# kianoosh-j/CL_MultiView_Stereo

Hardware: AMD Instinct MI355X
Metric: Mpix/s depth (1080p, 128 depth hyp, 5 views) + depth L1 vs ref (higher is better)
Workload: dtype i8 (NCC: 8-bit intensities as int8 v_dot4 operands, i32 window sums, f32 costs; SLIC / superpixel SAD / refinement in f32 with the reference's f64 promotions)

## Files before the change

cl_multiview_stereo_amd/csrc/launch_plan.cpp:

```cpp
#include "launch_plan.h"

#include <algorithm>
#include <climits>
#include <cmath>
#include <cstdlib>
#include <cstring>

extern char** environ;

namespace mvs {
namespace plan {

Tuning plan_tuning() {
  Tuning t;
  bool any = false;
  for (char** e = environ; e && *e && !any; e++) {
    const char* s = *e;
    any = s[0] == 'M' && s[1] == 'V' && s[2] == 'S' && s[3] == '_' && (s[4] == 'S' || s[4] == 'F');
  }
  if (!any) return t;
  const auto num = [](const char* name, int dflt) {
    const char* e = getenv(name);
    return e ? atoi(e) : dflt;
  };
  const auto is = [](const char* name, const char* value) {
    const char* e = getenv(name);
    return e && !strcmp(e, value);
  };
  const int wps = num("MVS_SWEEP_WPS", 0);
  t.sweep_wps = (wps == 1 || wps == 2 || wps == 4) ? wps : 0;
  t.sweep_transpose = num("MVS_SWEEP_TRANSPOSE", 2);
  t.sweep_hz = num("MVS_SWEEP_HZ", 1) != 0;
  t.sweep_ring = num("MVS_SWEEP_RING", 1) != 0;
  if (const char* kv = getenv("MVS_SAD_KERNEL")) {
    t.sad_kernel = kv;
    t.sad_named = true;
  }
  t.sad_aff = getenv("MVS_SAD_AFF") == nullptr;
  t.filter_px = is("MVS_FILTER_KERNEL", "px");
  t.filter_fb_q = num("MVS_FILTER_FB", 2);
  t.filter_fb_px = num("MVS_FILTER_FB", 4);
  t.filter_ns = num("MVS_FILTER_NS", 2);
  t.filter_bound = num("MVS_FILTER_BOUND", 1) != 0;
  t.filter_ref_order = is("MVS_FILTER_ORDER", "ref");
  t.slic_tiles9 = num("MVS_SLIC_TILES9", 0) == 1;
  t.slic_update_walk = num("MVS_SLIC_UPDATE", 1) != 0;
  return t;
}

SlicPlan plan_slic(const Tuning& t, int V, int W, int H, int S, int no_iter, int edge_enable, int search,
                   int enforce_connectivity) {
  SlicPlan p;
  p.V = V, p.W = W, p.H = H, p.S = S;
  const int mw = p.mw = map_dim(W, S), mh = p.mh = map_dim(H, S);
  float xy = 1.0f / (1.4242f * (float)S);
  float col = 15.0f / (1.7321f * 128.0f);
  p.xy = xy * xy;
  p.col = col * col;
  const bool tiles = S % kLocal == 0;
  const int cpl = p.cpl = S * 3 / kLocal;
  const int G = p.G = tiles ? cpl * cpl : (int)__builtin_ceilf((float)(S * S * 9) / (float)(kLocal * kLocal));
  const int ntx = p.ntx = (W + 15) / 16, nty = p.nty = (H + 15) / 16;
  const size_t P = (size_t)V * W * H;
  const bool l16 = !tiles && no_iter > 0 && (long)mw * mh <= 65536;
  size_t sb = tiles ? sizeof(float) * 6 * (size_t)G * mw * mh * V : 0;
  if (enforce_connectivity || edge_enable) sb = std::max(sb, sizeof(uint32_t) * P);
  if (l16) sb = std::max(sb, sizeof(uint16_t) * P);
  p.scratch_bytes = sb;

  p.steps.reserve(6 + 2 * (size_t)no_iter);
  const auto step = [&p](SlicKernel k, unsigned gx, unsigned gy, unsigned gz, unsigned block) -> SlicStep& {
    p.steps.push_back(SlicStep{k, 0, 0, 0, 0, 0, {gx, gy, gz}, block, false, false, false, false});
    return p.steps.back();
  };
  const unsigned cx = (mw + 63) / 64, px = (W + 255) / 256;
  step(kSlicInitCenters, cx, mh, V, 64);
  if (edge_enable == 1 || edge_enable == 2) {
    step(kSlicEdge, px, H, V, 256);
    if (edge_enable == 1)
      step(kSlicEdgeStore, (unsigned)std::min<long>(((long)P + 255) / 256, 8192), 1, 1, 256);
    else
      step(kSlicApplyEdge, cx, mh, V, 64);
  }
  const bool tiles4 = !search && (S == 32 || S == 64) && (long)W * H * 16 < (1L << 31) &&
                      (long)mw * mh * G * 24 < (1L << 31) && !t.slic_tiles9;
  const auto assign = [&](bool more) {
    if (tiles) {
      SlicStep& s = tiles4 ? step(kSlicAssignTiles4, (ntx + 3) / 4, nty, V, 256)
                           : step(kSlicAssignTiles9, (ntx * nty + 3) / 4, V, 1, 256);
      if (tiles4)
        s.S16 = S / 16;
      else
        s.S3 = search;
      s.labels = !more, s.part = more;
    } else {
      SlicStep& s = step(kSlicAssign, (W + kAssignTW - 1) / kAssignTW, (H + kAssignTH - 1) / kAssignTH, V, 256);
      s.S3 = search;
      s.labels = !(more && l16), s.lb16 = more && l16;
    }
  };
  const bool walk = (long)W * H * 16 < (1L << 31) && t.slic_update_walk;
  assign(no_iter > 0);
  for (int i = 0; i < no_iter; i++) {
    if (tiles) {
      step(kSlicUpdateFinalize, (mw * mh + 31) / 32, V, 1, 256).CPL = cpl == 6 ? 6 : 0;
    } else {
      SlicStep& s = step(walk ? kSlicUpdateWalk : kSlicUpdate, (mw * mh + 3) / 4, V, 1, 256);
      s.UT = G > 4 ? 4 : 1;
      s.LT = l16 ? 16 : 32;
    }
    assign(i + 1 < no_iter);
  }
  if (enforce_connectivity) {
    step(kSlicSuppress, px, H, V, 256).to_scratch = true;
    step(kSlicSuppress, px, H, V, 256);
  }
  return p;
}

SpixlSweepPlan plan_sweep_spixl(const Tuning& t, int V, int W, int H, int S, int D, const float* levels,
                                const int* vs, const int* sn, int aw, int z0, int z1, bool allow_relayout) {
  SpixlSweepPlan p;
  if (z1 <= z0) return p;
  if ((long)(W + H) * H * 16 >= (1L << 31)) {
    p.err = "superpixel sweep: image too large for 32-bit offsets";
    return p;
  }
  p.launch = true;
  p.mw = map_dim(W, S);
  p.mh = map_dim(H, S);
  const long M = (long)p.mw * p.mh;
  const bool half = D <= 32;
  int wps = (D + 63) / 64;
  wps = wps >= 3 ? 4 : wps;
  const int wps_env = half ? 0 : t.sweep_wps;
  if (wps_env) wps = wps_env;
  const int tmode = t.sweep_transpose;
  p.tstride = H;
  if (tmode > 0 && allow_relayout) {
    std::vector<int32_t> slot(4 * (size_t)V, -1);
    long units = 0;
    for (int z = z0; z < z1; z++)
      for (int k = 0; k < sn[z]; k++) {
        const int v = vs[(size_t)V * z + k];
        if (v < 0 || v >= V) continue;
        const int dx = v % aw - z % aw, dy = v / aw - z / aw;
        const int kind = dx == 0 ? 1 : tmode < 2 ? 0 : dx == dy ? 2 : dx == -dy ? 3 : 0;
        if (kind && slot[4 * v + kind] < 0 && units + W + H <= INT32_MAX) {
          slot[4 * v + kind] = (int32_t)units;
          units += kind == 1 ? W : W + H - 1;
        }
      }
    if (units > 0) {
      for (int v = 0; v < V; v++)
        for (int kind = 1; kind < 4; kind++)
          if (slot[4 * v + kind] >= 0) p.relayouts.push_back({v, kind, slot[4 * v + kind]});
      p.slot = std::move(slot);
      p.units = units;
    }
  }
  const bool relaid = p.units > 0;
  bool hz = !relaid && t.sweep_hz;
  for (int z = z0; z < z1 && hz; z++)
    for (int k = 0; k < sn[z] && hz; k++) {
      const int v = vs[(size_t)V * z + k];
      if (v / aw != z / aw) hz = false;
      const float fdxv = (float)(v % aw - z % aw);
      for (int l = 0; l < D && hz; l++) {
        const float f = levels[l] * fdxv;
        if (!(fabsf(f) < 16777216.0f) || f != truncf(f)) hz = false;
      }
    }
  bool ring = hz && !half && t.sweep_ring;
  if (ring) {
    float rng = 0.0f;
    for (int c0 = 0; c0 < D; c0 += 64) {
      float lo = levels[c0], hi = lo;
      for (int l = c0; l < std::min(D, c0 + 64); l++) {
        lo = std::min(lo, levels[l]);
        hi = std::max(hi, levels[l]);
      }
      rng = std::max(rng, hi - lo);
    }
    int mdx = 0;
    for (int z = z0; z < z1; z++)
      for (int k = 0; k < sn[z]; k++) mdx = std::max(mdx, std::abs(vs[(size_t)V * z + k] % aw - z % aw));
// ... 139 lines not shown
```

cl_multiview_stereo_amd/csrc/launch_plan.h:

```cpp
#pragma once
#include <cstddef>
#include <cstdint>
#include <string>
#include <vector>

namespace mvs {

inline int map_dim(int n, int S) {
  return (int)__builtin_ceilf((float)n / (float)S);
}

constexpr int kLocal = 16;
constexpr int kAssignTW = 64, kAssignTH = 16;

constexpr int kSwU = 336;

constexpr int SB_TW = 60;
constexpr int SB_NBLK = 2;
struct SadArgs {
  int W, H, D, nn, z;
  int tiles_x, ntiles, tiles_per_xcd, nch;
  int bw, brows;
};
struct alignas(16) SadRec {
  int view, sxmin, sxmax, pad0;
  float fdymin, fdymax;
  int pad1[2];
  int sx[16];
  float fdy[16];
};
static_assert(sizeof(SadRec) == 160, "SadRec is uploaded as 40 int32 words");
constexpr int PT = 32;

constexpr int kFilterRG = 4;

namespace plan {

struct Tuning {
  bool slic_tiles9 = false;
  bool slic_update_walk = true;
  int sweep_wps = 0;
  int sweep_transpose = 2;
  bool sweep_hz = true;
  bool sweep_ring = true;
  std::string sad_kernel = "auto";
  bool sad_named = false;
  bool sad_aff = true;
  bool filter_px = false;
  int filter_fb_q = 2;
  int filter_fb_px = 4;
  int filter_ns = 2;
  bool filter_bound = true;
  bool filter_ref_order = false;
};
Tuning plan_tuning();

enum SlicKernel {
  kSlicInitCenters, kSlicEdge, kSlicEdgeStore, kSlicApplyEdge,
  kSlicAssign,
  kSlicAssignTiles9,
  kSlicAssignTiles4,
  kSlicUpdateFinalize,
  kSlicUpdateWalk,
  kSlicUpdate,
  kSlicSuppress
};
struct SlicStep {
  SlicKernel kernel;
  int S3, S16, CPL, UT, LT;
  unsigned grid[3], block;
  bool labels;
  bool lb16;
  bool part;
  bool to_scratch;
};
struct SlicPlan {
  int V = 0, W = 0, H = 0, S = 0;
  int mw = 0, mh = 0;
  float xy = 0, col = 0;
  int G = 0, cpl = 0, ntx = 0, nty = 0;
  size_t scratch_bytes = 0;
  std::vector<SlicStep> steps;
};
SlicPlan plan_slic(const Tuning& t, int V, int W, int H, int S, int no_iter, int edge_enable, int search,
                   int enforce_connectivity);

constexpr int kSweepGeneral = 0, kSweepHzGather = 1, kSweepHzRing = 2, kSweepRelaid = 3;
struct SpixlRelayout {
  int view, kind, slot;
};
struct SpixlSweepPlan {
  const char* err = nullptr;
  bool launch = false;
  int form = 0, lps = 64, wps = 1;
  int mw = 0, mh = 0;
  unsigned grid_x = 0, grid_y = 0;
  std::vector<int32_t> slot;
  std::vector<SpixlRelayout> relayouts;
  long units = 0, tstride = 0;
  int last[5] = {0, 0, 0, 0, 0};
};
SpixlSweepPlan plan_sweep_spixl(const Tuning& t, int V, int W, int H, int S, int D, const float* levels,
                                const int* vs, const int* sn, int aw, int z0, int z1, bool allow_relayout);

struct SadPlan {
  bool band = false;
  int TH = 0, PPW = 0, AFF = 0, BWT = 0;
  std::vector<int32_t> table;
  SadArgs args{};
  size_t lds = 0;
  unsigned grid_x = 0, grid_y = 1;
  std::string err;
};
bool sad_band_geometry(int DC, int RR, bool aff, int V, int W, int H, int D, const float* levels, const int* vs,
                       const int* sn, int aw, float bl, int z, SadPlan& p);
SadPlan plan_sad(const Tuning& t, int V, int W, int H, int D, const float* levels, const int* vs, const int* sn,
                 int aw, float bl, int z);

enum FilterKernel { kFilterNone, kFilterSel8, kFilterPx16_8, kFilterQ, kFilterPx32, kFilterSel64, kFilterPlain };
struct FilterPlan {
  FilterKernel kernel = kFilterNone;
  int FB = 0, NS = 0, ROWB = 0, RM = 0;
  int inb = 0;
  unsigned grid[3] = {0, 1, 1}, block = 256;
  long PP = 0;
  long proj_off = 0;
};
FilterPlan plan_remove_incons(const Tuning& t, int V, int W, int H, int aw, int z0, int z1, int ya, int yb,
                              bool band);

}
}
```

cl_multiview_stereo_amd/csrc/sweep.hip:

```cpp
#include <algorithm>
#include <cmath>
#include <cstdlib>
#include <cstring>
#include <vector>

#include "mvs_internal.h"

namespace mvs {
namespace {

__global__ __launch_bounds__(256) void k_boundary(const float* __restrict__ spixl,
                                                  const uint32_t* __restrict__ labels, int W, int H, int S, int mw,
                                                  int mh, uint8_t* __restrict__ rep) {
  const int lane = threadIdx.x & 63;
  const long s = (long)blockIdx.x * 4 + (threadIdx.x >> 6);
  const int z = blockIdx.y;
  const long M = (long)mw * mh, P = (long)W * H;
  if (s >= M) return;
  const float* sp = spixl + 8 * (z * M + s);
  int cx = (int)sp[1], cy = (int)sp[2];
  if (cx < S) cx += (S - cx);
  if (cx + S > W) cx -= S;
  if (cy < S) cy += (S - cy);
  if (cy + S > H) cy -= S;
  const uint32_t id = (uint32_t)s;
  const uint32_t* L = labels + z * P;
  const int k = lane >> 3, j = lane & 7;
  const int dx = k < 3 ? -1 : (k < 5 ? 0 : 1);
  const int dy = (k == 0 || k == 3 || k == 5) ? -1 : ((k == 1 || k == 6) ? 0 : 1);
  int d = 0;
  for (int i0 = 1; i0 < S; i0 += 32) {
    uint32_t v[4];
    bool in[4];
#pragma unroll
    for (int m = 0; m < 4; m++) {
      const int i = i0 + j + 8 * m, xx = cx + dx * i, yy = cy + dy * i;
      in[m] = i < S && xx >= 0 && xx < W && yy >= 0 && yy < H;
      v[m] = L[in[m] ? (long)yy * W + xx : 0];
    }
#pragma unroll
    for (int m = 0; m < 4; m++)
      if (in[m] && v[m] == id) d = i0 + j + 8 * m - 1;
  }
  d = max(d, __shfl_xor(d, 1));
  d = max(d, __shfl_xor(d, 2));
  d = max(d, __shfl_xor(d, 4));
  uint32_t w = (uint32_t)(d & 0xff) << (8 * (k & 3));
  w |= __shfl_xor(w, 8);
  w |= __shfl_xor(w, 16);
  const uint32_t hi = __shfl(w, 32);
  if (lane == 0) *(uint2*)(rep + 8 * (z * M + s)) = make_uint2(w, hi);
}

typedef __attribute__((address_space(3))) void* lds_vptr_t;
typedef const __attribute__((address_space(1))) void* glb_vptr_t;
__device__ __forceinline__ void glds16(const void* src, void* dst) {
  __builtin_amdgcn_global_load_lds((glb_vptr_t)src, (lds_vptr_t)dst, 16, 0, 0);
}

struct SweepArgs {
  int V, W, H, mw, mh, D, aw, z;
  float bl;
};

typedef unsigned u32x3 __attribute__((ext_vector_type(3)));
typedef float f32x4 __attribute__((ext_vector_type(4)));
__device__ __forceinline__ float tap_ad(const float4& A, const u32x3& bv) {
  float t0, t1, t2, r;
  asm("v_sub_f32 %0, %1, %2" : "=v"(t0) : "v"(A.x), "v"(__uint_as_float(bv.x)));
  asm("v_sub_f32 %0, %1, %2" : "=v"(t1) : "v"(A.y), "v"(__uint_as_float(bv.y)));
  asm("v_add_f32 %0, |%1|, |%2|" : "=v"(r) : "v"(t0), "v"(t1));
  asm("v_sub_f32 %0, %1, %2" : "=v"(t2) : "v"(A.z), "v"(__uint_as_float(bv.z)));
  asm("v_add_f32 %0, %1, |%2|" : "=v"(r) : "v"(r), "v"(t2));
  return r;
}
__device__ __forceinline__ float tap_acc(float val, float ad, bool in) {
  float v30, t;
  asm("v_add_f32 %0, 0x41f00000, %1" : "=v"(v30) : "v"(val));
  asm("v_add_f32 %0, 0xc1f00000, %1" : "=v"(t) : "v"(v30));
  asm("v_add_f32 %0, %1, %2" : "=v"(t) : "v"(t), "v"(ad));
  return in ? t : v30;
}
template <int LPS, bool TL, bool HZ = false>
__global__ __launch_bounds__(256) void k_sweep_spixl(const float4* __restrict__ lab, float* __restrict__ spixl,
                                                     const uint8_t* __restrict__ rep,
                                                     const float* __restrict__ levels, const int* __restrict__ vs,
                                                     const int* __restrict__ sn, SweepArgs a, int wps,
                                                     const float4* __restrict__ labT,
                                                     const int* __restrict__ tslot, long tstride) {
  __shared__ float4 refc[8][25];
  __shared__ float2 refxy[8][25];
  __shared__ float wbest[4];
  __shared__ int wbi[4];
  const int lane = threadIdx.x & 63, w = threadIdx.x >> 6;
  const int ll = lane & (LPS - 1);
  const int spb = LPS == 64 ? 4 / wps : 8, h = LPS == 64 ? w % wps : 0;
  const int slot = LPS == 64 ? w / wps : 2 * w + (lane >> 5);
  const int z = a.z + blockIdx.y;
  const long M = (long)a.mw * a.mh, P = (long)a.W * a.H;
  const long nb = (M + spb - 1) / spb, per = (nb + 7) / 8;
  const long blk = (long)(blockIdx.x & 7) * per + (blockIdx.x >> 3);
  const long s = blk * spb + slot;
  const bool active = blk < nb && s < M && slot < spb;
  const long idx = z * M + (active ? s : 0);
  const uint8_t* dr = rep + 8 * idx;
  int bl_ = max((int)dr[0], max((int)dr[1], (int)dr[2]));
  int br_ = max((int)dr[5], max((int)dr[6], (int)dr[7]));
  int bt_ = max((int)dr[0], max((int)dr[3], (int)dr[5]));
  int bb_ = max((int)dr[2], max((int)dr[4], (int)dr[7]));
  float stx = (float)fmax(1.0, 0.25 * (double)(float)(bl_ + br_));
  float sty = (float)fmax(1.0, 0.25 * (double)(float)(bt_ + bb_));
  float cx = spixl[8 * idx + 1], cy = spixl[8 * idx + 2];
  const float4* labz = lab + (long)z * P;
  if (ll < 25 && (LPS == 32 || h == 0)) {
    int i = ll / 5 - 2, j = ll % 5 - 2;
    int xr = (int)(cx + (float)i * stx);
    int yr = (int)(cy + (float)j * sty);
    bool in = xr >= 0 && yr >= 0 && xr < a.W && yr < a.H;
    if (HZ)
      refxy[slot][ll] = make_float2(__int_as_float(in ? xr : -(1 << 30)), __int_as_float(in ? yr * a.W : 0));
    else
      refxy[slot][ll] = make_float2(in ? (float)xr : -1.0e9f, (float)yr);
    refc[slot][ll] = in ? labz[(long)yr * a.W + xr] : make_float4(0.f, 0.f, 0.f, 0.f);
  }
  __syncthreads();
  int rx = z % a.aw, ry = z / a.aw;
  int nn = sn[z];
  float best = 1000000.0f;
  int bi = 0x7fffffff;
  for (int dl = ll + LPS * h; dl < a.D; dl += LPS * wps) {
    float d = levels[dl];
    float mn = 1000000.0f;
    for (int n = 0; n < nn; n++) {
      int view = vs[a.V * z + n];
      int vx = view % a.aw, vy = view / a.aw;
      float fdx = d * (float)(vx - rx);
      float fdy = (a.bl * d) * (float)(vy - ry);
      const int ddx = vx - rx, ddy = vy - ry;
      if (HZ) {
        const int sh = (int)fdx;
        const __amdgpu_buffer_rsrc_t rs =
            __builtin_amdgcn_make_buffer_rsrc((void*)(lab + (long)view * P), 0, (int)(P * 16), 0x00020000);
        float val = 0.0f;
#pragma unroll 5
        for (int t = 0; t < 25; t++) {
          const float2 rf = refxy[slot][t];
          const int xp = __float_as_int(rf.x) - sh;
          const bool in = (unsigned)xp < (unsigned)a.W;
          const unsigned bo = (unsigned)(__float_as_int(rf.y) + xp) << 4;
          const u32x3 bv = __builtin_amdgcn_raw_buffer_load_b96(rs, (int)bo, 0, 0);
          val = tap_acc(val, tap_ad(refc[slot][t], bv), in);
        }
        if (val < mn) mn = val;
        continue;
      }
      const int kind = !TL ? 0 : ddx == 0 ? 1 : ddx == ddy ? 2 : ddx == -ddy ? 3 : 0;
      const int ts = TL && kind ? tslot[4 * view + kind] : -1;
      const float4* labv = TL && ts >= 0 ? labT + (long)ts * tstride : lab + (long)view * P;
      const __amdgpu_buffer_rsrc_t rs = __builtin_amdgcn_make_buffer_rsrc((void*)labv, 0, 0x7fffffff, 0x00020000);
      const int sxs = !TL || ts < 0 ? 1 : a.H;
      const int sys = !TL || ts < 0 ? a.W : kind == 1 ? 1 : kind == 2 ? 1 - a.H : a.H + 1;
      const int off = TL && ts >= 0 && kind == 2 ? (a.H - 1) * a.H : 0;
      float val = 0.0f;
#pragma unroll 5
      for (int t = 0; t < 25; t++) {
        const float2 r = refxy[slot][t];
        const int xp = (int)(r.x - fdx);
        const int yp = (int)(r.y - fdy);
        const bool in = (unsigned)xp < (unsigned)a.W && (unsigned)yp < (unsigned)a.H;
        const int bo = in ? (off + yp * sys + xp * sxs) * 16 : 0;
        const u32x3 bv = __builtin_amdgcn_raw_buffer_load_b96(rs, bo, 0, 0);
        const float3 B = make_float3(__uint_as_float(bv.x), __uint_as_float(bv.y), __uint_as_float(bv.z));
        const float4 A = refc[slot][t];
        float ad = fabsf(A.x - B.x) + fabsf(A.y - B.y);
        ad = ad + fabsf(A.z - B.z);
        const float v30 = val + 30.0f;
        val = in ? (v30 - 30.0f) + ad : v30;
      }
      if (val < mn) mn = val;
    }
    if (mn < best) {
      best = mn;
      bi = dl;
    }
  }
#pragma unroll
  for (int o = LPS / 2; o >= 1; o >>= 1) {
    float ob = __shfl_xor(best, o, 64);
    int oi = __shfl_xor(bi, o, 64);
    if (ob < best || (ob == best && oi < bi)) {
      best = ob;
      bi = oi;
    }
  }
  if (LPS == 32) {
    if (active && ll == 0) spixl[8 * idx + 7] = (bi != 0x7fffffff && best < 1000000.0f) ? levels[bi] : 0.0f;
    return;
  }
  if (lane == 0) {
    wbest[w] = best;
    wbi[w] = bi;
  }
  __syncthreads();
  if (active && h == 0 && lane == 0) {
    for (int k = 1; k < wps; k++) {
      const float ob = wbest[w + k];
      const int oi = wbi[w + k];
      if (ob < best || (ob == best && oi < bi)) {
        best = ob;
        bi = oi;
      }
    }
    spixl[8 * idx + 7] = (bi != 0x7fffffff && best < 1000000.0f) ? levels[bi] : 0.0f;
  }
}

__device__ __forceinline__ void wait_vm(int n) {
  switch (n) {
    case 0: __builtin_amdgcn_s_waitcnt(0x0f70); break;
    case 1: __builtin_amdgcn_s_waitcnt(0x0f71); break;
    case 2: __builtin_amdgcn_s_waitcnt(0x0f72); break;
    case 3: __builtin_amdgcn_s_waitcnt(0x0f73); break;
    case 4: __builtin_amdgcn_s_waitcnt(0x0f74); break;
    case 5: __builtin_amdgcn_s_waitcnt(0x0f75); break;
    default: __builtin_amdgcn_s_waitcnt(0x0f76); break;
  }
}
__device__ __forceinline__ float wave_min_f(float v) {
  v = fminf(v, __shfl_xor(v, 32));
  v = fminf(v, __shfl_xor(v, 16));
  v = fminf(v, __shfl_xor(v, 8));
  v = fminf(v, __shfl_xor(v, 4));
  v = fminf(v, __shfl_xor(v, 2));
  v = fminf(v, __shfl_xor(v, 1));
  return __int_as_float(__builtin_amdgcn_readfirstlane(__float_as_int(v)));
}
template <int WPS>
__global__ __launch_bounds__(256) void k_sweep_spixl_ring(const float4* __restrict__ lab, float* __restrict__ spixl,
                                                          const uint8_t* __restrict__ rep,
                                                          const float* __restrict__ levels, const int* __restrict__ vs,
                                                          const int* __restrict__ sn, SweepArgs a) {
  constexpr int SPB = 4 / WPS;
  __shared__ __align__(16) float4 ring[4][2][kSwU];
  __shared__ float4 refc[SPB][25];
  __shared__ int rxr[SPB][5], ryr[SPB][5];
  __shared__ unsigned rvm[SPB];
  __shared__ float wbest[4];
  __shared__ int wbi[4];
  const int lane = threadIdx.x & 63, w = __builtin_amdgcn_readfirstlane(threadIdx.x >> 6);
  const int h = w % WPS, slot = w / WPS;
  const int z = a.z + blockIdx.y;
  const long M = (long)a.mw * a.mh, P = (long)a.W * a.H;
  const long nbk = (M + SPB - 1) / SPB, per = (nbk + 7) / 8;
  const long blk = (long)(blockIdx.x & 7) * per + (blockIdx.x >> 3);
  const long s = blk * SPB + slot;
  const bool active = blk < nbk && s < M;
  const long idx = z * M + (active ? s : 0);
  if (h == 0) {
    const uint8_t* dr = rep + 8 * idx;
    const int bl_ = max((int)dr[0], max((int)dr[1], (int)dr[2]));
    const int br_ = max((int)dr[5], max((int)dr[6], (int)dr[7]));
    const int bt_ = max((int)dr[0], max((int)dr[3], (int)dr[5]));
    const int bb_ = max((int)dr[2], max((int)dr[4], (int)dr[7]));
    const float stx = (float)fmax(1.0, 0.25 * (double)(float)(bl_ + br_));
    const float sty = (float)fmax(1.0, 0.25 * (double)(float)(bt_ + bb_));
    const float cx = spixl[8 * idx + 1], cy = spixl[8 * idx + 2];
    const int i = lane / 5 - 2, j = lane % 5 - 2;
    const int xr = (int)(cx + (float)i * stx);
    const int yr = (int)(cy + (float)j * sty);
    const bool in = lane < 25 && xr >= 0 && yr >= 0 && xr < a.W && yr < a.H;
    if (lane < 25) {
      float4 rc = in ? lab[(long)z * P + (long)yr * a.W + xr] : make_float4(0.f, 0.f, 0.f, 0.f);
      rc.w = __int_as_float(in ? xr : -(1 << 30));
      refc[slot][lane] = rc;
      if (j == -2) rxr[slot][i + 2] = xr;
      if (i == -2) ryr[slot][j + 2] = yr;
    }
    const unsigned long long bal = __ballot(in);
    if (lane == 0) rvm[slot] = (unsigned)bal;
  }
  __syncthreads();
  const unsigned vm = __builtin_amdgcn_readfirstlane(rvm[slot]);
  int xr[5], yr[5];
#pragma unroll
  for (int q = 0; q < 5; q++) {
    xr[q] = rxr[slot][q];
    yr[q] = ryr[slot][q];
  }
  int xlo = 1 << 30, xhi = -(1 << 30);
#pragma unroll
  for (int q = 0; q < 5; q++)
    if ((vm >> (5 * q)) & 0x1fu) {
      xlo = min(xlo, xr[q]);
      xhi = max(xhi, xr[q]);
    }
  const int rx = z % a.aw;
  int rcol[25];
#pragma unroll
  for (int t = 0; t < 25; t++) rcol[t] = __float_as_int(refc[slot][t].w);
  const unsigned ring_base = (unsigned)(uintptr_t)(lds_vptr_t)&ring[w][0][0];
  const unsigned refc_base = (unsigned)(uintptr_t)(lds_vptr_t)&refc[slot][0];
  const int nn = sn[z];
  float best = 1000000.0f;
  int bi = 0x7fffffff;
  for (int p0 = 64 * h; p0 < a.D; p0 += 64 * WPS) {
    const int dl = p0 + lane;
    const bool act = dl < a.D;
    const float d = levels[act ? dl : a.D - 1];
    const float dlo = wave_min_f(d), dhi = -wave_min_f(-d);
    auto window = [&](int n, int& ulo, int& U, int& sh) {
      const int view = vs[a.V * z + n];
      const float fdx = (float)(view % a.aw - rx);
      sh = (int)(d * fdx);
      const int s0 = (int)(dlo * fdx), s1 = (int)(dhi * fdx);
      const int shmin = min(s0, s1), shmax = max(s0, s1);
      ulo = max(xlo - shmax, 0);
      U = min(xhi - shmin, a.W - 1) - ulo + 1;
    };
    auto stage = [&](int n, int j, int k, int ulo, int U) -> int {
      if (U <= 0 || !((vm >> j) & 0x108421u)) return 0;
      U = min(U, kSwU);
      const int view = vs[a.V * z + n];
      const float4* row = lab + (long)view * P + (long)yr[j] * a.W + ulo;
      const int np = (U + 63) >> 6;
      for (int q = 0; q < np; q++) {
        const int c0 = U >= 64 ? min(q * 64, U - 64) : 0;
        glds16(row + min(c0 + lane, U - 1), &ring[w][k & 1][c0]);
      }
      return np;
    };
    float mn = 1000000.0f;
    if (nn > 0) {
      int ulo0, U0, sh0;
      window(0, ulo0, U0, sh0);
      int pcn = stage(0, 0, 0, ulo0, U0);
      pcn = stage(0, 1, 1, ulo0, U0);
      int ulo_c = ulo0, sh_c = sh0;
      int ulo_s = ulo0, U_s = U0;
      for (int n = 0; n < nn; n++) {
        float ad[25];
#pragma unroll
        for (int j = 0; j < 5; j++) {
          const int k = 5 * n + j;
          wait_vm(k + 1 < 5 * nn ? pcn : 0);
          int xp[5];
          unsigned ra[5];
#pragma unroll
          for (int i = 0; i < 5; i++) {
            xp[i] = rcol[i * 5 + j] - sh_c;
            const bool in = (unsigned)xp[i] < (unsigned)a.W;
            ra[i] = ring_base + (unsigned)(k & 1) * (kSwU * 16u) + (in ? (unsigned)(xp[i] - ulo_c) * 16u : 0u);
          }
          const unsigned rb = refc_base + (unsigned)j * 16u;
          u32x3 Bv[5];
          f32x4 Av[5];
          asm volatile(
              "ds_read_b96 %0, %10\n\t"
              "ds_read_b96 %1, %11\n\t"
              "ds_read_b96 %2, %12\n\t"
              "ds_read_b96 %3, %13\n\t"
              "ds_read_b96 %4, %14\n\t"
              "ds_read_b128 %5, %15\n\t"
              "ds_read_b128 %6, %15 offset:80\n\t"
              "ds_read_b128 %7, %15 offset:160\n\t"
              "ds_read_b128 %8, %15 offset:240\n\t"
              "ds_read_b128 %9, %15 offset:320\n\t"
              "s_waitcnt lgkmcnt(0)"
              : "=&v"(Bv[0]), "=&v"(Bv[1]), "=&v"(Bv[2]), "=&v"(Bv[3]), "=&v"(Bv[4]), "=&v"(Av[0]), "=&v"(Av[1]),
                "=&v"(Av[2]), "=&v"(Av[3]), "=&v"(Av[4])
              : "v"(ra[0]), "v"(ra[1]), "v"(ra[2]), "v"(ra[3]), "v"(ra[4]), "v"(rb)
              : "memory");
#pragma unroll
          for (int i = 0; i < 5; i++) {
            const bool in = (unsigned)xp[i] < (unsigned)a.W;
            const float v = tap_ad(make_float4(Av[i].x, Av[i].y, Av[i].z, 0.f), Bv[i]);
            ad[5 * i + j] = in ? v : -1.0f;
          }
          const int k2 = k + 2;
          int pc2 = 0;
          if (k2 < 5 * nn) {
            const int n2 = k2 / 5, j2 = k2 - 5 * n2;
            if (j2 == 0) {
              int sh2;
              window(n2, ulo_s, U_s, sh2);
            }
            pc2 = stage(n2, j2, k2, ulo_s, U_s);
          }
          pcn = pc2;
        }
        float val = 0.0f;
#pragma unroll
        for (int t = 0; t < 25; t++) val = tap_acc(val, ad[t], ad[t] >= 0.0f);
        mn = val < mn ? val : mn;
        if (n + 1 < nn) {
          ulo_c = ulo_s;
          const int view = vs[a.V * z + n + 1];
          sh_c = (int)(d * (float)(view % a.aw - rx));
        }
      }
    }
    if (act && mn < best) {
      best = mn;
      bi = dl;
    }
  }
#pragma unroll
  for (int o = 32; o >= 1; o >>= 1) {
    const float ob = __shfl_xor(best, o, 64);
    const int oi = __shfl_xor(bi, o, 64);
    if (ob < best || (ob == best && oi < bi)) {
      best = ob;
      bi = oi;
    }
  }
  if (lane == 0) {
    wbest[w] = best;
    wbi[w] = bi;
  }
  __syncthreads();
  if (active && h == 0 && lane == 0) {
    for (int k = 1; k < WPS; k++) {
      const float ob = wbest[w + k];
      const int oi = wbi[w + k];
      if (ob < best || (ob == best && oi < bi)) {
        best = ob;
        bi = oi;
      }
    }
    spixl[8 * idx + 7] = (bi != 0x7fffffff && best < 1000000.0f) ? levels[bi] : 0.0f;
  }
}

constexpr float SB_INIT = 1000000.0f;
constexpr int SB_NOROW = -0x40000000;

static_assert(sizeof(SadRec) == 160, "k_sad_band reads one 160-byte record per step");

struct SadBand {
  int bx0, by0, nrows, ncols;
};
template <int TH>
__device__ __forceinline__ SadBand sad_band_of(const SadRec& e, int x0, int y0, int W, int H) {
  SadBand g;
  g.bx0 = min(max(x0 - 2 - e.sxmax, 0), W - 1);
  const int bx1 = min(max(x0 + SB_TW + 1 - e.sxmin, 0), W - 1);
  g.by0 = min(max((int)((float)(y0 - 2) - e.fdymax), 0), H - 1);
  const int by1 = min(max((int)((float)(y0 + TH + 1) - e.fdymin), 0), H - 1);
  g.nrows = by1 - g.by0 + 1;
  g.ncols = bx1 - g.bx0 + 1;
  return g;
}

typedef float f32x2 __attribute__((ext_vector_type(2)));


template <int TH, int PPW, bool AFF = false, int BWT = 0>
__global__ __launch_bounds__(256) void k_sad_band(const float4* __restrict__ lab, const float* __restrict__ levels,
                                                  const SadRec* __restrict__ plan, SadArgs a,
                                                  float* __restrict__ disp) {
  constexpr int RR = TH + 4, DC = 8 * PPW;
  extern __shared__ __align__(16) uint8_t smem[];
  float4* band = (float4*)smem;
  int* rtab = (int*)(band + 2 * a.brows * a.bw);
  const int tid = threadIdx.x, lane = tid & 63, wave = __builtin_amdgcn_readfirstlane(tid >> 6);
  const int bid = blockIdx.x, grp = bid & 7;
  const int tile = grp * a.tiles_per_xcd + (bid >> 3);
  if (tile >= a.ntiles) return;
  const int W = a.W, H = a.H;
  const int x0 = (tile % a.tiles_x) * SB_TW, y0 = (tile / a.tiles_x) * TH;
  const long P = (long)W * H;
  const int gx = x0 - 2 + lane;
  const bool gxok = gx >= 0 && gx < W;
  float rL[RR], ra[RR], rb[RR];
  {
    const float4* labz = lab + (long)a.z * P;
#pragma unroll
    for (int r = 0; r < RR; r++) {
      const int gy = y0 - 2 + r;
      const bool in = gxok && gy >= 0 && gy < H;
      const float4 c = labz[in ? (long)gy * W + gx : 0];
      rL[r] = c.x;
      ra[r] = c.y;
      rb[r] = c.z;
    }
  }
// ... 262 lines not shown
          }
      }
#pragma unroll
      for (int o = 0; o < 4; o++)
        if (val[o] < mn[o]) mn[o] = val[o];
    }
#pragma unroll
    for (int o = 0; o < 4; o++)
      if (mn[o] < cost[o]) {
        cost[o] = mn[o];
        dsp[o] = d;
      }
  }
#pragma unroll
  for (int o = 0; o < 4; o++) {
    int x = x0 + tx, y = y0 + ty0 + o;
    if (x < a.W && y < a.H) disp[(long)y * a.W + x] = dsp[o];
  }
}

struct Top4 {
  float v0 = 1000000.0f, v1 = 1000000.0f, v2 = 1000000.0f, v3 = 1000000.0f;
  int i0 = -1, i1 = -1, i2 = -1, i3 = -1;
  __device__ __forceinline__ void insert(float cc, int ci) {
    if (cc < v3) {
      if (cc < v2) {
        v3 = v2; i3 = i2;
        if (cc < v1) {
          v2 = v1; i2 = i1;
          if (cc < v0) { v1 = v0; i1 = i0; v0 = cc; i0 = ci; }
          else { v1 = cc; i1 = ci; }
        } else { v2 = cc; i2 = ci; }
      } else { v3 = cc; i3 = ci; }
    }
  }
  __device__ __forceinline__ void emit(const float* levels, float* disp, float* conf, long p) const {
    disp[p] = i0 >= 0 ? levels[i0] : 0.0f;
    if (conf) {
      float c2 = 1000000.0f;
      if (i1 >= 0 && (i1 < i0 - 1 || i1 > i0 + 1)) c2 = v1;
      else if (i2 >= 0 && (i2 < i0 - 1 || i2 > i0 + 1)) c2 = v2;
      else if (i3 >= 0 && (i3 < i0 - 1 || i3 > i0 + 1)) c2 = v3;
      conf[p] = (i0 < 0 || c2 == 1000000.0f) ? 0.0f : c2 - v0;
    }
  }
};

template <int NP, int UNR>
__global__ __launch_bounds__(256) void k_wta(const float* __restrict__ vol, const float* __restrict__ levels, long P,
                                             int D, float* __restrict__ disp, float* __restrict__ conf) {
  typedef float vec __attribute__((ext_vector_type(NP)));
  const long p = (blockIdx.x * (long)blockDim.x + threadIdx.x) * NP;
  if (p >= P) return;
  Top4 t[NP];
  const vec* col = (const vec*)(vol + p);
  const long Pv = P / NP;
  int dl = 0;
  for (; dl + UNR <= D; dl += UNR) {
    vec c[UNR];
#pragma unroll
    for (int u = 0; u < UNR; u++) c[u] = __builtin_nontemporal_load(col + (long)(dl + u) * Pv);
#pragma unroll
    for (int u = 0; u < UNR; u++)
#pragma unroll
      for (int k = 0; k < NP; k++) t[k].insert(c[u][k], dl + u);
  }
  for (; dl < D; dl++) {
    const vec c = col[(long)dl * Pv];
#pragma unroll
    for (int k = 0; k < NP; k++) t[k].insert(c[k], dl);
  }
#pragma unroll
  for (int k = 0; k < NP; k++) t[k].emit(levels, disp, conf, p + k);
}

}

int launch_boundary(hipStream_t s, int V, int W, int H, int S, const float* spixl, const uint32_t* labels,
                    uint8_t* rep) {
  int mw = map_dim(W, S), mh = map_dim(H, S);
  hipLaunchKernelGGL(k_boundary, dim3((mw * mh + 3) / 4, V), dim3(256), 0, s, spixl, labels, W, H, S, mw, mh, rep);
  MVS_LAUNCH_CHECK("k_boundary");
  return 0;
}

template <int KIND>
__global__ __launch_bounds__(256) void k_relayout_lab(const float4* __restrict__ lab, int W, int H, int view,
                                                      float4* __restrict__ out) {
  __shared__ float4 t[32][33];
  const int x0 = blockIdx.x * 32, y0 = blockIdx.y * 32, tx = threadIdx.x & 31, ty = threadIdx.x >> 5;
  const float4* src = lab + (long)view * W * H;
#pragma unroll
  for (int k = 0; k < 4; k++) {
    const int y = y0 + ty + 8 * k, x = x0 + tx;
    if (x < W && y < H) t[ty + 8 * k][tx] = src[(long)y * W + x];
  }
  __syncthreads();
  if (KIND == 1) {
#pragma unroll
    for (int k = 0; k < 4; k++) {
      const int x = x0 + ty + 8 * k, y = y0 + tx;
      if (x < W && y < H) out[(long)x * H + y] = t[tx][ty + 8 * k];
    }
    return;
  }
  for (int d0 = 0; d0 < 63; d0 += 8) {
    const int dd = d0 + ty, yl = tx;
    const int xl = KIND == 2 ? yl + dd - 31 : dd - yl;
    const int x = x0 + xl, y = y0 + yl;
    if (dd < 63 && xl >= 0 && xl < 32 && x < W && y < H)
      out[KIND == 2 ? (long)(x - y + H - 1) * H + y : (long)(x + y) * H + y] = t[yl][xl];
  }
}

int launch_sweep_spixl(mvs_ctx* ctx, int V, int W, int H, int S, const float* lab, float* spixl,
                       const uint8_t* rep, const float* levels, int D, const int* vs, const int* sn, int aw,
                       float bl, int z0, int z1) {
  const plan::Tuning t = plan::plan_tuning();
  const auto planned = [&](bool relayout) {
    return plan::plan_sweep_spixl(t, V, W, H, S, D, ctx->h_levels.data(), ctx->h_vs.data(), ctx->h_sn.data(), aw, z0,
                                  z1, relayout);
  };
  plan::SpixlSweepPlan p = planned(true);
  if (p.err) return arg_fail(p.err);
  if (!p.launch) return 0;
  hipStream_t s = ctx->stream;
  const float4* labT = nullptr;
  const int* tslot = nullptr;
  if (p.units > 0) {
    int rc = 0;
    float4* buf = (float4*)scratch(ctx, (size_t)p.units * p.tstride * sizeof(float4), &rc);
    if (rc == MVS_E_NOMEM) {
      (void)hipGetLastError();
      p = planned(false);
    } else if (rc) {
      return rc;
    } else {
      tslot = plan_upload(ctx, p.slot, &rc);
      if (rc) return rc;
      labT = buf;
      const dim3 tg((W + 31) / 32, (H + 31) / 32);
      static constexpr void (*relayout[3])(const float4*, int, int, int, float4*) = {k_relayout_lab<1>, k_relayout_lab<2>,
                                                                                     k_relayout_lab<3>};
      for (const plan::SpixlRelayout& r : p.relayouts)
        hipLaunchKernelGGL(relayout[r.kind - 1], tg, dim3(256), 0, s, (const float4*)lab, W, H, r.view,
                           buf + (long)r.slot * p.tstride);
      MVS_LAUNCH_CHECK("k_relayout_lab");
    }
  }
  SweepArgs a{V, W, H, p.mw, p.mh, D, aw, z0, bl};
  const dim3 g(p.grid_x, p.grid_y);
  if (p.form == plan::kSweepHzRing) {
    static constexpr void (*ring[3])(const float4*, float*, const uint8_t*, const float*, const int*, const int*,
                                     SweepArgs) = {k_sweep_spixl_ring<1>, k_sweep_spixl_ring<2>, k_sweep_spixl_ring<4>};
    hipLaunchKernelGGL(ring[p.wps == 1 ? 0 : p.wps == 2 ? 1 : 2], g, dim3(256), 0, s, (const float4*)lab, spixl, rep,
                       levels, vs, sn, a);
    MVS_LAUNCH_CHECK("k_sweep_spixl_ring");
  } else {
    const bool half = p.lps == 32;
    const auto kern = p.form == plan::kSweepRelaid     ? (half ? k_sweep_spixl<32, true> : k_sweep_spixl<64, true>)
                      : p.form == plan::kSweepHzGather ? (half ? k_sweep_spixl<32, false, true> : k_sweep_spixl<64, false, true>)
                                                       : (half ? k_sweep_spixl<32, false> : k_sweep_spixl<64, false>);
    hipLaunchKernelGGL(kern, g, dim3(256), 0, s, (const float4*)lab, spixl, rep, levels, vs, sn, a, p.wps, labT, tslot,
                       p.tstride);
    MVS_LAUNCH_CHECK("k_sweep_spixl");
  }
  std::copy(p.last, p.last + 5, ctx->sweep_last);
  return 0;
}

namespace {
using SadBandKernel = void (*)(const float4*, const float*, const SadRec*, SadArgs, float*);
SadBandKernel sad_band_kernel(const plan::SadPlan& p) {
  static constexpr SadBandKernel k[2][3] = {
      {k_sad_band<8, 2>, k_sad_band<8, 2, true, 64>, k_sad_band<8, 2, true, 128>},
      {k_sad_band<8, 1>, k_sad_band<8, 1, true, 64>, k_sad_band<8, 1, true, 128>}};
  return k[p.PPW == 1][!p.AFF ? 0 : p.BWT == 64 ? 1 : 2];
}
}

int launch_sweep_pixel_sad(mvs_ctx* ctx, int V, int W, int H, const float* lab, const float* levels_host, int D,
                           const int* vs_host, const int* sn_host, int aw, float bl, int z0, int z1, float* disp) {
  const plan::Tuning t = plan::plan_tuning();
  const long P = (long)W * H;
  for (int z = z0; z < z1; z++) {
    float* out = disp + (long)(z - z0) * P;
    const plan::SadPlan p = plan::plan_sad(t, V, W, H, D, levels_host, vs_host, sn_host, aw, bl, z);
    if (!p.err.empty()) {
      set_error(p.err);
      return MVS_E_UNSUPPORTED;
    }
    const dim3 g(p.grid_x, p.grid_y);
    if (p.band) {
      int rc = 0;
      const int32_t* dev = plan_upload(ctx, p.table, &rc);
      if (rc) return rc;
      const SadBandKernel kern = sad_band_kernel(p);
      MVS_HIP(raise_lds(ctx, (const void*)kern, p.lds), "hipFuncSetAttribute(sad lds)");
      hipLaunchKernelGGL(kern, g, dim3(256), p.lds, ctx->stream, (const float4*)lab, ctx->d_levels,
                         (const SadRec*)dev, p.args, out);
      MVS_LAUNCH_CHECK("k_sad_band");
    } else {
      SweepArgs a{V, W, H, W, H, D, aw, z, bl};
      hipLaunchKernelGGL(k_sweep_pixel_sad, g, dim3(256), 0, ctx->stream, (const float4*)lab, ctx->d_levels,
                         ctx->d_vs, ctx->d_sn, a, out);
      MVS_LAUNCH_CHECK("k_sweep_pixel_sad");
    }
  }
  return 0;
}

int launch_wta(hipStream_t s, int W, int H, int D, const float* vol, const float* levels, float* disp,
               float* conf) {
  long P = (long)W * H;
  hipLaunchKernelGGL((k_wta<1, 16>), dim3((unsigned)((P + 255) / 256)), dim3(256), 0, s, vol, levels, P, D, disp,
                     conf);
  MVS_LAUNCH_CHECK("k_wta");
  return 0;
}

}
```

Baseline: 6088.

## Add fast all-in-bounds path to ring sweep with buffer-to-LDS loads and compile-time waits

Adds a specialized path in the superpixel ring sweep kernel for superpixels whose 25 taps are all valid. It loads rows into LDS with raw buffer-load-to-LDS using precomputed per-neighbour descriptors and offsets. Wave-uniform coordinates are hoisted to scalars, vmcnt waits become compile-time constants via a switch over page count, and LDS reads are batched in inline asm. This aims to cut address arithmetic and wait overhead in the staged-row pipeline, at the cost of code size, register pressure and a second code path that can be disabled by an env knob.

```diff
diff --git a/cl_multiview_stereo_amd/csrc/launch_plan.cpp b/cl_multiview_stereo_amd/csrc/launch_plan.cpp
--- a/cl_multiview_stereo_amd/csrc/launch_plan.cpp
+++ b/cl_multiview_stereo_amd/csrc/launch_plan.cpp
@@ -32,6 +32,7 @@
   t.sweep_transpose = num("MVS_SWEEP_TRANSPOSE", 2);
   t.sweep_hz = num("MVS_SWEEP_HZ", 1) != 0;
   t.sweep_ring = num("MVS_SWEEP_RING", 1) != 0;
+  t.sweep_ring_fast = num("MVS_SWEEP_RING_FAST", 1) != 0;
   if (const char* kv = getenv("MVS_SAD_KERNEL")) {
     t.sad_kernel = kv;
     t.sad_named = true;
diff --git a/cl_multiview_stereo_amd/csrc/launch_plan.h b/cl_multiview_stereo_amd/csrc/launch_plan.h
--- a/cl_multiview_stereo_amd/csrc/launch_plan.h
+++ b/cl_multiview_stereo_amd/csrc/launch_plan.h
@@ -43,6 +43,7 @@
   int sweep_transpose = 2;
   bool sweep_hz = true;
   bool sweep_ring = true;
+  bool sweep_ring_fast = true;
   std::string sad_kernel = "auto";
   bool sad_named = false;
   bool sad_aff = true;
diff --git a/cl_multiview_stereo_amd/csrc/sweep.hip b/cl_multiview_stereo_amd/csrc/sweep.hip
--- a/cl_multiview_stereo_amd/csrc/sweep.hip
+++ b/cl_multiview_stereo_amd/csrc/sweep.hip
@@ -2,6 +2,7 @@
 #include <cmath>
 #include <cstdlib>
 #include <cstring>
+#include <type_traits>
 #include <vector>
 
 #include "mvs_internal.h"
@@ -226,6 +227,19 @@
     default: __builtin_amdgcn_s_waitcnt(0x0f76); break;
   }
 }
+template <int N>
+__device__ __forceinline__ void wait_vm_imm() {
+  static_assert(N >= 0 && N <= 15, "vmcnt's low field");
+  __builtin_amdgcn_s_waitcnt(0x0f70 | N);
+}
+constexpr int kSwP = (kSwU + 63) / 64;
+struct RingNb {
+  int ulo, np;
+  int sh;
+  __amdgpu_buffer_rsrc_t rs;
+  int c0[kSwP];
+  int vo[kSwP];
+};
 __device__ __forceinline__ float wave_min_f(float v) {
   v = fminf(v, __shfl_xor(v, 32));
   v = fminf(v, __shfl_xor(v, 16));
@@ -239,7 +253,7 @@
 __global__ __launch_bounds__(256) void k_sweep_spixl_ring(const float4* __restrict__ lab, float* __restrict__ spixl,
                                                           const uint8_t* __restrict__ rep,
                                                           const float* __restrict__ levels, const int* __restrict__ vs,
-                                                          const int* __restrict__ sn, SweepArgs a) {
+                                                          const int* __restrict__ sn, SweepArgs a, int fast) {
   constexpr int SPB = 4 / WPS;
   __shared__ __align__(16) float4 ring[4][2][kSwU];
   __shared__ float4 refc[SPB][25];
@@ -301,6 +315,14 @@
   const unsigned ring_base = (unsigned)(uintptr_t)(lds_vptr_t)&ring[w][0][0];
   const unsigned refc_base = (unsigned)(uintptr_t)(lds_vptr_t)&refc[slot][0];
   const int nn = sn[z];
+  int xs[5], ys[5];
+#pragma unroll
+  for (int q = 0; q < 5; q++) {
+    xs[q] = __builtin_amdgcn_readfirstlane(xr[q]);
+    ys[q] = __builtin_amdgcn_readfirstlane(yr[q]);
+  }
+  const int xlo_s = __builtin_amdgcn_readfirstlane(xlo), xhi_s = __builtin_amdgcn_readfirstlane(xhi);
+  const bool all_in = fast && vm == 0x1ffffffu;
   float best = 1000000.0f;
   int bi = 0x7fffffff;
   for (int p0 = 64 * h; p0 < a.D; p0 += 64 * WPS) {
@@ -330,7 +352,110 @@
       return np;
     };
     float mn = 1000000.0f;
-    if (nn > 0) {
+    if (all_in) {
+      using rt_np = std::integral_constant<int, -1>;
+      const auto nb_of = [&](int n) __attribute__((always_inline)) {
+        RingNb b;
+        const int view = vs[a.V * z + n];
+        const float fdx = (float)(view % a.aw - rx);
+        b.sh = (int)(d * fdx);
+        const int s0 = (int)(dlo * fdx), s1 = (int)(dhi * fdx);
+        const int shmin = min(s0, s1), shmax = max(s0, s1);
+        b.ulo = max(xlo_s - shmax, 0);
+        const int U = min(min(xhi_s - shmin, a.W - 1) - b.ulo + 1, kSwU);
+        b.np = U > 0 ? (U + 63) >> 6 : 0;
+        b.rs = __builtin_amdgcn_make_buffer_rsrc((void*)(lab + (long)view * P), 0, (int)(P * 16), 0x00020000);
+#pragma unroll
+        for (int q = 0; q < kSwP; q++) {
+          b.c0[q] = U >= 64 ? min(q * 64, U - 64) : 0;
+          b.vo[q] = min(b.c0[q] + lane, U - 1) * 16;
+        }
+        return b;
+      };
+      const auto stage_row = [&](const RingNb& b, int j, int sl, auto npc) __attribute__((always_inline)) {
+        constexpr int NPC = decltype(npc)::value;
+        const int so = (ys[j] * a.W + b.ulo) * 16;
+#pragma unroll
+        for (int q = 0; q < kSwP; q++)
+          if (NPC >= 0 ? q < NPC : q < b.np)
+            __builtin_amdgcn_raw_ptr_buffer_load_lds(b.rs, (lds_vptr_t)&ring[w][sl][b.c0[q]], 16, b.vo[q], so, 0, 0);
+      };
+      const auto neighbour = [&](const RingNb& c, const RingNb& nx, bool more, int par, auto npc)
+                                 __attribute__((always_inline)) -> float {
+        constexpr int NP = decltype(npc)::value;
+        bool in[5];
+        unsigned ra[2][5];
+#pragma unroll
+        for (int i = 0; i < 5; i++) {
+          const int xp = xs[i] - c.sh;
+          in[i] = (unsigned)xp < (unsigned)a.W;
+          const unsigned off = in[i] ? (unsigned)(xp - c.ulo) * 16u : 0u;
+          ra[0][i] = ring_base + (unsigned)par * (kSwU * 16u) + off;
+          ra[1][i] = ring_base + (unsigned)(par ^ 1) * (kSwU * 16u) + off;
+        }
+        float ad[25];
+#pragma unroll
+        for (int j = 0; j < 5; j++) {
+          if (j < 4)
+            wait_vm_imm<NP>();
+          else
+            wait_vm(more ? nx.np : 0);
+          const unsigned rb = refc_base + (unsigned)j * 16u;
+          u32x3 Bv[5];
+          f32x4 Av[5];
+          asm volatile(
+              "ds_read_b96 %0, %10\n\t"
+              "ds_read_b96 %1, %11\n\t"
+              "ds_read_b96 %2, %12\n\t"
+              "ds_read_b96 %3, %13\n\t"
+              "ds_read_b96 %4, %14\n\t"
+              "ds_read_b128 %5, %15\n\t"
+              "ds_read_b128 %6, %15 offset:80\n\t"
+              "ds_read_b128 %7, %15 offset:160\n\t"
+              "ds_read_b128 %8, %15 offset:240\n\t"
+              "ds_read_b128 %9, %15 offset:320\n\t"
+              "s_waitcnt lgkmcnt(0)"
+              : "=&v"(Bv[0]), "=&v"(Bv[1]), "=&v"(Bv[2]), "=&v"(Bv[3]), "=&v"(Bv[4]), "=&v"(Av[0]), "=&v"(Av[1]),
+                "=&v"(Av[2]), "=&v"(Av[3]), "=&v"(Av[4])
+              : "v"(ra[j & 1][0]), "v"(ra[j & 1][1]), "v"(ra[j & 1][2]), "v"(ra[j & 1][3]), "v"(ra[j & 1][4]), "v"(rb)
+              : "memory");
+#pragma unroll
+          for (int i = 0; i < 5; i++) ad[5 * i + j] = tap_ad(make_float4(Av[i].x, Av[i].y, Av[i].z, 0.f), Bv[i]);
+          if (j < 3)
+            stage_row(c, j + 2, (par + j) & 1, npc);
+          else if (more)
+            stage_row(nx, j - 3, (par + j) & 1, rt_np{});
+        }
+        float val = 0.0f;
+#pragma unroll
+        for (int i = 0; i < 5; i++)
+#pragma unroll
+          for (int j = 0; j < 5; j++) val = tap_acc(val, ad[5 * i + j], in[i]);
+        return val;
+      };
+      if (nn > 0) {
+        RingNb cur = nb_of(0);
+        stage_row(cur, 0, 0, rt_np{});
+        stage_row(cur, 1, 1, rt_np{});
+        for (int n = 0; n < nn; n++) {
+          const bool more = n + 1 < nn;
+          const RingNb nx = nb_of(more ? n + 1 : n);
+          const int par = n & 1;
+          float val;
+          switch (cur.np) {
+            case 0: val = neighbour(cur, nx, more, par, std::integral_constant<int, 0>{}); break;
+            case 1: val = neighbour(cur, nx, more, par, std::integral_constant<int, 1>{}); break;
+            case 2: val = neighbour(cur, nx, more, par, std::integral_constant<int, 2>{}); break;
+            case 3: val = neighbour(cur, nx, more, par, std::integral_constant<int, 3>{}); break;
+            case 4: val = neighbour(cur, nx, more, par, std::integral_constant<int, 4>{}); break;
+            case 5: val = neighbour(cur, nx, more, par, std::integral_constant<int, 5>{}); break;
+            default: val = neighbour(cur, nx, more, par, std::integral_constant<int, kSwP>{}); break;
+          }
+          mn = val < mn ? val : mn;
+          cur = nx;
+        }
+      }
+    } else if (nn > 0) {
       int ulo0, U0, sh0;
       window(0, ulo0, U0, sh0);
       int pcn = stage(0, 0, 0, ulo0, U0);
@@ -899,9 +1024,9 @@
   const dim3 g(p.grid_x, p.grid_y);
   if (p.form == plan::kSweepHzRing) {
     static constexpr void (*ring[3])(const float4*, float*, const uint8_t*, const float*, const int*, const int*,
-                                     SweepArgs) = {k_sweep_spixl_ring<1>, k_sweep_spixl_ring<2>, k_sweep_spixl_ring<4>};
+                                     SweepArgs, int) = {k_sweep_spixl_ring<1>, k_sweep_spixl_ring<2>, k_sweep_spixl_ring<4>};
     hipLaunchKernelGGL(ring[p.wps == 1 ? 0 : p.wps == 2 ? 1 : 2], g, dim3(256), 0, s, (const float4*)lab, spixl, rep,
-                       levels, vs, sn, a);
+                       levels, vs, sn, a, (int)t.sweep_ring_fast);
     MVS_LAUNCH_CHECK("k_sweep_spixl_ring");
   } else {
     const bool half = p.lps == 32;
```

After: 6145, median of 6. Within noise of the previous version (+0.9%).
